# codyheiser/MILWRM

Hardware: AMD Instinct MI355X
Metric: pixels/sec (node) for preprocess+k-means fit+label, 30-ch MxIF k=8; %HBM peak (higher is better)
Workload: dtype f32 (fp64 accumulation)

## Files before the change

### include/milwrm_amd.h

```cpp
#ifndef MILWRM_AMD_H
#define MILWRM_AMD_H

#include <stddef.h>
#include <stdint.h>

#ifdef __cplusplus
extern "C" {
#endif

#define MW_OK 0
#define MW_EINVAL (-1)
#define MW_EHIP (-2)
#define MW_EUNSUPPORTED (-3)

#define MW_U8 0
#define MW_U16 1
#define MW_F32 2

int mw_version(void);
const char* mw_last_error(void);
int mw_stream_blocks(int64_t n);
int64_t mw_rows_per_block(int64_t n);

size_t mw_nz_stats_ws_bytes(int64_t n_pix, int C);
// ... 172 lines not shown
int mw_col_absmax(const float* d_X, int64_t S, int F, float* d_out, void* stream);
int mw_col_absmax_acc(const float* d_X, int64_t S, int F, float* d_out, void* stream);

int mw_kmeans_fit_history(int64_t* out, int cap);

size_t mw_kmeans_fit_ws_bytes(int64_t S, int F, int k);
int mw_kmeans_fit(const float* d_X, int64_t S, int F, const double* h_mu,
                  const double* h_inv, const double* h_feature_var, const float* h_xmax,
                  int k, const double* h_init, uint32_t seed, int max_iter, double tol,
                  uint8_t* d_labels, double* h_centers, double* h_inertia, int* h_n_iter,
                  int64_t* h_init_idx, void* d_ws, size_t ws_bytes, void* stream);
int mw_kmeans_fit_async(const float* d_X, int64_t S, int F, const double* h_mu,
                        const double* h_inv, const double* h_feature_var, const float* h_xmax,
                        int k, const double* h_init, uint32_t seed, int max_iter, double tol,
                        uint8_t* d_labels, double* h_centers, int* h_n_iter, int64_t* h_init_idx,
                        void* d_ws, size_t ws_bytes, double* h_final_rec, int* h_inertia_exp,
                        void* stream);
int mw_kmeans_fit_async_moments(const float* d_X, int64_t S, int F, const double* h_mu,
                                const double* h_inv, const double* h_feature_var, const float* h_xmax,
                                int k, const double* h_init, uint32_t seed, int max_iter, double tol,
                                uint8_t* d_labels, double* h_centers, int* h_n_iter, int64_t* h_init_idx,
                                void* d_ws, size_t ws_bytes, double* h_final_rec, int* h_inertia_exp,
                                int n_seg, const mw_kpp_seg* h_segs, void* stream);

int mw_lloyd_fits(const float* d_X, int64_t S, int F, const float* d_a32, const float* d_b32,
                  const int32_t* d_qexp, const float* h_a32, const float* h_b32,
                  const int32_t* h_qexp, const float* h_xmax, const double* h_mu,
                  const double* h_inv, int n, const int* h_k, const double* h_init,
                  uint8_t* const* d_labels, float* const* d_ub, float* const* d_lb,
                  void* const* d_ws, float* d_par, double* d_out, int max_iter, double tol,
                  int first_kind, int queue_kind, double queue_below, int dense_min,
                  int nobound, double* h_centers, double* h_inertia, int* h_n_iter,
                  int64_t* h_hist, int hist_cap, int* h_hist_len, double* h_timing,
                  void* stream);

typedef struct mw_fit_comm {
  void* ctx;
  int world;
  int rank;
  int64_t rows_total;
  int64_t row_offset;
  double* d_msg;
  int64_t msg_len;
  int (*all_reduce_sum)(void* ctx, int64_t off, int64_t n, void* stream);
  int (*all_gather)(void* ctx, int64_t in_off, int64_t n, int64_t out_off, void* stream);
} mw_fit_comm;
// ... 66 lines not shown
```

### milwrm_amd/_native.py

```python
from __future__ import annotations

import ctypes as C
import os
import threading

import torch

_HERE = os.path.dirname(os.path.abspath(__file__))
LIB_PATH = os.environ.get("MW_LIB") or os.path.join(_HERE, "libmilwrm_amd.so")

MW_U8, MW_U16, MW_F32 = 0, 1, 2
_EINVAL, _EHIP, _EUNSUP = -1, -2, -3

_lib = None
_lock = threading.Lock()

c_i64, c_i32, c_u32, c_u64 = C.c_int64, C.c_int, C.c_uint32, C.c_uint64
c_f32, c_sz, c_vp = C.c_float, C.c_size_t, C.c_void_p
c_dp = C.POINTER(C.c_double)

_PROTOS = {
    "mw_version": (c_i32, []),
    "mw_host_labels_f64": (c_i32, [c_vp, c_i64, c_vp, c_i32]),
    "mw_host_f32_to_f64": (c_i32, [c_vp, c_i64, c_vp, c_i32]),
# ... 52 lines not shown
                                 c_vp, c_vp, c_vp, c_vp, c_vp, c_vp, c_vp, c_vp, c_vp]),
    "mw_kpp_fold_rec_bytes": (c_sz, [c_i64, c_i32, c_i32]),
    "mw_kpp_fold_supported": (c_i32, [c_i32, c_i32, c_i32]),
    "mw_kmeans_fit_history": (c_i32, [c_vp, c_i32]),
    "mw_kpp_best_ptr": (c_vp, [c_vp, c_i64, c_i32]),
    "mw_kpp_pots": (c_i32, [c_vp, c_i64, c_i32, c_i32, c_vp, c_vp]),
    "mw_kpp_search": (c_i32, [c_vp, c_i64, c_i32, c_vp, c_i32, c_i32, c_i32, c_vp, c_vp, c_vp]),
    "mw_kpp_trial": (c_i32, [c_vp, c_i64, c_i32, c_vp, c_vp, c_i32, c_i32, c_vp, c_i32, c_vp, c_vp]),
    "mw_lloyd_ws_bytes": (c_sz, [c_i64, c_i32, c_i32]),
    "mw_lloyd_ws_bytes_kinds": (c_sz, [c_i64, c_i32, c_i32, c_i32]),
    "mw_lloyd_list_moved": (c_i32, [c_vp, c_vp, c_i64, c_i32, c_i32, c_vp, c_vp]),
    "mw_lloyd_rec_len": (c_i32, [c_i32, c_i32]),
    "mw_lloyd_pass": (c_i32, [c_vp, c_i64, c_i32, c_vp, c_vp, c_vp, c_i32, c_vp, c_i32, c_i32, c_vp]),
    "mw_col_absmax": (c_i32, [c_vp, c_i64, c_i32, c_vp, c_vp]),
    "mw_col_absmax_acc": (c_i32, [c_vp, c_i64, c_i32, c_vp, c_vp]),
    "mw_kmeans_fit_ws_bytes": (c_sz, [c_i64, c_i32, c_i32]),
    "mw_kmeans_fit": (c_i32, [c_vp, c_i64, c_i32, c_vp, c_vp, c_vp, c_vp, c_i32, c_vp, c_u32, c_i32,
                              C.c_double, c_vp, c_vp, c_vp, c_vp, c_vp, c_vp, c_sz, c_vp]),
    "mw_kmeans_fit_async": (c_i32, [c_vp, c_i64, c_i32, c_vp, c_vp, c_vp, c_vp, c_i32, c_vp, c_u32, c_i32,
                                    C.c_double, c_vp, c_vp, c_vp, c_vp, c_vp, c_sz, c_vp, c_vp, c_vp]),
    "mw_kmeans_fit_async_moments": (c_i32, [c_vp, c_i64, c_i32, c_vp, c_vp, c_vp, c_vp, c_i32, c_vp, c_u32, c_i32,
                                            C.c_double, c_vp, c_vp, c_vp, c_vp, c_vp, c_sz, c_vp, c_vp, c_i32,
                                            c_vp, c_vp]),
    "mw_lloyd_fits": (c_i32, [c_vp, c_i64, c_i32, c_vp, c_vp, c_vp, c_vp, c_vp, c_vp, c_vp, c_vp, c_vp,
                              c_i32, c_vp, c_vp, c_vp, c_vp, c_vp, c_vp, c_vp, c_vp, c_i32, C.c_double,
                              c_i32, c_i32, C.c_double, c_i32, c_i32, c_vp, c_vp, c_vp, c_vp, c_i32, c_vp,
                              c_vp, c_vp]),
    "mw_lloyd_fits_msg_len": (c_i64, [c_i64, c_i32, c_i32]),
    "mw_lloyd_fits_sharded": (c_i32, [c_vp, c_i64, c_i32, c_vp, c_vp, c_vp, c_vp, c_vp, c_vp, c_vp, c_vp, c_vp,
                                      c_i32, c_vp, c_vp, c_vp, c_vp, c_vp, c_vp, c_vp, c_vp, c_i32, C.c_double,
                                      c_i32, c_i32, C.c_double, c_i32, c_i32, c_vp, c_vp, c_vp, c_vp, c_i32,
                                      c_vp, c_vp, c_vp, c_vp]),
    "mw_farthest_ws_bytes": (c_sz, [c_i64]),
    "mw_farthest": (c_i32, [c_vp, c_i64, c_i32, c_vp, c_vp, c_vp, c_i32, c_vp, c_i32, c_vp, c_vp, c_vp, c_vp]),
    "mw_assign_ws_bytes": (c_sz, [c_i64, c_i32]),
    "mw_assign_conf": (c_i32, [c_vp, c_i32, c_vp, c_i32, c_vp, c_vp, c_vp, c_i32, c_vp, c_i64, c_vp, c_vp, c_vp, c_vp]),
    "mw_assign_reduce": (c_i32, [c_vp, c_i64, c_i32, c_vp, c_vp]),
    "mw_domain_sse_ws_bytes": (c_sz, [c_i64, c_i32, c_i32]),
    "mw_domain_sse_out_len": (c_i32, [c_i32, c_i32]),
    "mw_domain_sse": (c_i32, [c_vp, c_i32, c_vp, c_i32, c_vp, c_vp, c_vp, c_vp, c_vp, c_i32, c_i32, c_vp,
                              c_i64, c_vp, c_i32, c_vp, c_vp]),
    "mw_domain_sse_f64": (c_i32, [c_vp, c_i32, c_vp, c_i32, c_vp, c_vp, c_vp, c_vp, c_vp, c_i32, c_i32, c_vp,
                                  c_i64, c_vp, c_i32, c_vp, c_vp]),
    "mw_neighbor_mean": (c_i32, [c_vp, c_vp, c_i64, c_vp, c_i32, c_vp, c_vp]),
    "mw_col_stats_rows": (c_i32, [c_vp, c_i64, c_i32, c_vp, c_vp]),
    "mw_col_stats_absmax": (c_i32, [c_vp, c_i64, c_i32, c_vp, c_i32, c_vp]),
# ... 101 lines not shown
```

### milwrm_amd/csrc/fit.cpp

```cpp
#include <hip/hip_runtime.h>

#include <algorithm>
#include <chrono>
#include <cmath>
#include <cstring>
#include <limits>
#include <vector>

#include "common.h"

#pragma clang fp contract(off)

namespace mw {
void mt_init_genrand(uint32_t seed, uint32_t* mt);
void mt_regen(uint32_t* mt);

namespace {

struct LegacyRandom {
  uint32_t mt[624];
  int pos = 624;
  explicit LegacyRandom(uint32_t seed) { mt_init_genrand(seed, mt); }
  uint32_t next() {
    if (pos >= 624) { mt_regen(mt); pos = 0; }
    uint32_t y = mt[pos++];
    y ^= y >> 11;
    y ^= (y << 7) & 0x9D2C5680u;
    y ^= (y << 15) & 0xEFC60000u;
    y ^= y >> 18;
    return y;
  }
  double sample() {
    const uint32_t a = next() >> 5, b = next() >> 6;
    return (a * 67108864.0 + b) / 9007199254740992.0;
  }
};

double np_sum(const double* a, int64_t n) {
// ... 287 lines not shown
    return (e && e[0] == '0') ? 2 : 4;
  }();
  return q;
}
static FitLayout fit_layout(int64_t S, int F, int k) {
  const int T = 2 + (int)std::log((double)(k < 1 ? 1 : k));
  FitLayout L;
  L.small = 0;
  L.par = fal(64 * 4 * 4 + 64 * 8 * 2 + 64 * 64 * 8 + 64 * 8 * 2 + 130 * 8 + 64 * 8);
  L.ub = L.par + fal(((size_t)k * F + 2 * k) * 4);
  L.lb = L.ub + fal((size_t)S * 4);
  L.lws = L.lb + fal((size_t)S * 4);
  L.out = L.lws + fal(std::max(mw_lloyd_ws_bytes_kinds(S, k, F, lloyd_queue_kind() == 4),
                               mw_kpp_fold_rec_bytes(S, k, F)));
  L.big = L.out + fal((size_t)2 * mw_lloyd_rec_len(k, F) * 8);
  size_t big = mw_gather_ws_bytes(S, F);
  if (T <= 8) big = std::max(big, mw_kpp_ws_bytes(S, T));
  big = std::max(big, mw_farthest_ws_bytes(S));
  L.fold = L.big + fal(big);
  L.total = L.fold + fal(8192) + fal((size_t)S);
  return L;
}

}
}

using namespace mw;

extern "C" size_t mw_kmeans_fit_ws_bytes(int64_t S, int F, int k) {
  if (S <= 0 || F < 1 || F > 64 || k < 1 || k > 64) return 0;
  return fit_layout(S, F, k).total;
}

static int kmeans_fit_impl(const float* d_X, int64_t S, int F, const double* h_mu, const double* h_inv,
                           const double* h_feature_var, const float* h_xmax, int k, const double* h_init,
                           uint32_t seed, int max_iter, double tol, uint8_t* d_labels, double* h_centers,
                           double* h_inertia, int* h_n_iter, int64_t* h_init_idx, void* d_ws, size_t ws_bytes,
                           double* h_final_rec, int* h_inertia_exp, void* stream, int n_seg = 0,
                           const mw_kpp_seg* h_segs = nullptr);

static thread_local std::vector<int64_t> fit_hist;

extern "C" int mw_kmeans_fit_history(int64_t* out, int cap) {
  const int n = (int)(fit_hist.size() / 4);
  if (out)
    for (int i = 0; i < std::min(n, cap) * 4; ++i) out[i] = fit_hist[i];
  return n;
}

extern "C" int mw_kmeans_fit(const float* d_X, int64_t S, int F, const double* h_mu,
                             const double* h_inv, const double* h_feature_var, const float* h_xmax,
                             int k, const double* h_init, uint32_t seed, int max_iter, double tol,
                             uint8_t* d_labels, double* h_centers, double* h_inertia, int* h_n_iter,
                             int64_t* h_init_idx, void* d_ws, size_t ws_bytes, void* stream) {
  return kmeans_fit_impl(d_X, S, F, h_mu, h_inv, h_feature_var, h_xmax, k, h_init, seed, max_iter, tol,
                         d_labels, h_centers, h_inertia, h_n_iter, h_init_idx, d_ws, ws_bytes, nullptr, nullptr,
                         stream);
}

extern "C" int mw_kmeans_fit_async(const float* d_X, int64_t S, int F, const double* h_mu,
                                   const double* h_inv, const double* h_feature_var, const float* h_xmax,
                                   int k, const double* h_init, uint32_t seed, int max_iter, double tol,
// ... 2 lines not shown
                                   void* stream) {
  MW_CHECK_ARG(h_final_rec && h_inertia_exp, "mw_kmeans_fit_async: null final-record pointer");
  double unused = 0.0;
  return kmeans_fit_impl(d_X, S, F, h_mu, h_inv, h_feature_var, h_xmax, k, h_init, seed, max_iter, tol,
                         d_labels, h_centers, &unused, h_n_iter, h_init_idx, d_ws, ws_bytes, h_final_rec,
                         h_inertia_exp, stream);
}

extern "C" int mw_kmeans_fit_async_moments(const float* d_X, int64_t S, int F, const double* h_mu,
                                           const double* h_inv, const double* h_feature_var,
                                           const float* h_xmax, int k, const double* h_init, uint32_t seed,
                                           int max_iter, double tol, uint8_t* d_labels, double* h_centers,
                                           int* h_n_iter, int64_t* h_init_idx, void* d_ws, size_t ws_bytes,
                                           double* h_final_rec, int* h_inertia_exp, int n_seg,
                                           const mw_kpp_seg* h_segs, void* stream) {
  MW_CHECK_ARG(h_final_rec && h_inertia_exp, "mw_kmeans_fit_async_moments: null final-record pointer");
  MW_CHECK_ARG(n_seg == 0 || h_segs, "mw_kmeans_fit_async_moments: null segments");
  double unused = 0.0;
  return kmeans_fit_impl(d_X, S, F, h_mu, h_inv, h_feature_var, h_xmax, k, h_init, seed, max_iter, tol,
                         d_labels, h_centers, &unused, h_n_iter, h_init_idx, d_ws, ws_bytes, h_final_rec,
                         h_inertia_exp, stream, n_seg, h_segs);
}

static int kmeans_fit_impl(const float* d_X, int64_t S, int F, const double* h_mu, const double* h_inv,
                           const double* h_feature_var, const float* h_xmax, int k, const double* h_init,
                           uint32_t seed, int max_iter, double tol, uint8_t* d_labels, double* h_centers,
                           double* h_inertia, int* h_n_iter, int64_t* h_init_idx, void* d_ws, size_t ws_bytes,
                           double* h_final_rec, int* h_inertia_exp, void* stream, int n_seg,
                           const mw_kpp_seg* h_segs) {
  MW_CHECK_ARG(d_X && h_mu && h_inv && d_labels && h_centers && h_inertia && h_n_iter,
               "mw_kmeans_fit: null pointer");
  MW_CHECK_ARG(F >= 1 && F <= 64, "mw_kmeans_fit: F=%d outside [1, 64]", F);
  MW_CHECK_ARG(k >= 1 && k <= 64, "mw_kmeans_fit: n_clusters=%d outside [1, 64]", k);
  MW_CHECK_ARG(S >= k, "mw_kmeans_fit: n_samples=%lld should be >= n_clusters=%d", (long long)S, k);
  MW_CHECK_ARG(max_iter >= 1 && tol >= 0.0, "mw_kmeans_fit: bad max_iter / tol");
  const int T = 2 + (int)std::log((double)k);
  MW_CHECK_ARG(h_init || T <= 8, "mw_kmeans_fit: n_local_trials > 8");
  const FitLayout L = fit_layout(S, F, k);
  MW_CHECK_ARG(!d_ws || ws_bytes >= L.total, "mw_kmeans_fit: workspace %zu < %zu bytes", ws_bytes,
               L.total);
  hipStream_t st = as_stream(stream);
  DevBuf own;
  if (!d_ws) {
    MW_TRY(dev_alloc<char>(own, L.total));
    d_ws = own.p;
  }
  char* base = static_cast<char*>(d_ws);

  Fit fit;
  fit.S = S;
  fit.F = F;
  fit.k = k;
// ... 92 lines not shown

  std::vector<double> centers((size_t)k * F);
  if (h_init) {
    std::memcpy(centers.data(), h_init, centers.size() * sizeof(double));
  } else {
    LegacyRandom rs(seed);
    const double u0 = rs.sample();
    const int64_t first = first_center_index(S, u0);
    const bool moments = n_seg > 0 && k >= 2;
    std::vector<double> u(T);
    if (moments) {
      for (int t = 0; t < T; ++t) u[t] = rs.sample();
      MW_TRY(mw_kpp_init_moments(d_X, S, F, d_mu, d_inv, d_X + first * F, u.data(), T, n_seg, h_segs, big, st));
    } else {
      MW_TRY(mw_kpp_init(d_X, S, F, d_mu, d_inv, d_X + first * F, T, big, st));
    }
    for (int c = moments ? 2 : 1; c < k; ++c) {
      for (int t = 0; t < T; ++t) u[t] = rs.sample();
      if (fold && c == k - 1)
        MW_TRY(mw_kpp_step_fold(d_X, S, F, d_mu, d_inv, c, u.data(), T, big, first, fit.a32, fit.b32, fit.qexp,
                                d_labels, fit.ub, fit.lb, d_moved, base + L.fold, reinterpret_cast<double*>(fit.ws),
                                fit.out + fit.rl, st));
      else
        MW_TRY(mw_kpp_step(d_X, S, F, d_mu, d_inv, c, u.data(), T, big, st));
    }
    MW_TRY(mw_kpp_indices(big, S, T, k, d_idx, st));
    std::vector<int64_t> idx(k);
    if (fit.scaled_rows_dev(d_idx, first, k, h_mu, h_inv, reinterpret_cast<float*>(d_c64), centers,
                            idx.data()) == MW_OK) {
      if (h_init_idx) std::memcpy(h_init_idx, idx.data(), k * sizeof(int64_t));
    } else {
      MW_HIP(hipMemcpyAsync(idx.data(), d_idx, k * 8, hipMemcpyDeviceToHost, st));
      MW_HIP(hipStreamSynchronize(st));
      idx[0] = first;
      MW_TRY(fit.scaled_rows(idx.data(), k, h_mu, h_inv, centers));
      if (h_init_idx) std::memcpy(h_init_idx, idx.data(), k * sizeof(int64_t));
    }
  }

  fit_hist.clear();
  if (!fold) MW_HIP(hipMemsetAsync(d_labels, 255, (size_t)S, st));
  std::vector<int64_t> q_hi((size_t)k * F, 0), q_lo((size_t)k * F, 0), count(k, 0);
  std::vector<double> rec, cnew((size_t)k * F), weight(k), tmp(std::max(F, k));
  int64_t last_recomputed = -1;
  int n_iter = 0;
  bool done = false, strict = false;
  for (int it = 0; it < max_iter && !done; ++it) {
// ... 84 lines not shown
      } else {
        for (int f = 0; f < F; ++f) cnew[(size_t)j * F + f] = cnew[(size_t)amax * F + f];
      }
    }
    std::vector<double> shift2(k);
    for (int j = 0; j < k; ++j) {
      for (int f = 0; f < F; ++f) {
        const double d = cnew[(size_t)j * F + f] - centers[(size_t)j * F + f];
        tmp[f] = d * d;
      }
      const double sh = std::sqrt(np_sum(tmp.data(), F));
      shift2[j] = sh * sh;
    }
    centers.swap(cnew);
    n_iter = it + 1;
    if (changed == 0) {
      strict = done = true;
    } else if (np_sum(shift2.data(), k) <= tol_abs) {
      done = true;
    }
  }
  if (!done) n_iter = max_iter;

  std::vector<double> xs2(F), cn(k);
  for (int f = 0; f < F; ++f) {
    const double v = std::fabs(fit.a64[f]) * (double)xmax[f] + std::fabs(fit.b64[f]);
    xs2[f] = v * v;
  }
  const double xnorm = std::sqrt(np_sum(xs2.data(), F));
  double cmax = 0.0;
  for (int j = 0; j < k; ++j) {
    for (int f = 0; f < F; ++f) tmp[f] = centers[(size_t)j * F + f] * centers[(size_t)j * F + f];
    const double v = std::sqrt(np_sum(tmp.data(), F));
    cmax = j == 0 ? v : std::max(cmax, v);
  }
  const double xc = xnorm + cmax;
  const int iexp = exp_below(xc * xc * 1.01);
  MW_TRY(fit.upload(centers));
  fit_hist.insert(fit_hist.end(), {(int64_t)(strict ? 12 : 11), -1, -1, S});
  *h_n_iter = n_iter;
  std::memcpy(h_centers, centers.data(), centers.size() * sizeof(double));
  if (h_final_rec && !own.p && pinned_staging()) {
    MW_TRY(fit.pass_async(strict ? 2 : 1, 0, iexp, h_final_rec));
    *h_inertia_exp = iexp;
    hipEvent_t ev;
    MW_HIP(hipEventCreateWithFlags(&ev, hipEventDisableTiming));
    MW_HIP(hipEventRecord(ev, st));
    pin_busy = ev;
    *h_inertia = std::numeric_limits<double>::quiet_NaN();
    return MW_OK;
  }
  MW_TRY(fit.pass(strict ? 2 : 1, 0, iexp, rec));
  const double* tail = rec.data() + fit.rl - 4;
  *h_inertia = (tail[2] * 4294967296.0 + tail[3]) * std::ldexp(1.0, -iexp);
  if (h_final_rec) {
    std::memcpy(h_final_rec, rec.data(), (size_t)fit.rl * sizeof(double));
    *h_inertia_exp = iexp;
  }
  return MW_OK;
}

namespace mw {
namespace {

constexpr int kFitsMaxPerLaunch = 24;
constexpr int kKindFirst = 0, kKindTile = 1, kKindDense = 5;

struct FitsFit {
  int k = 0;
  std::vector<double> centers;
  std::vector<float> prev32;
  bool have_prev = false;
  std::vector<int64_t> q_hi, q_lo, count;
  bool done = false, strict = false, bounds_ok = true;
  int n_iter = 0;
  double drift_max = 0.0, prev_dmax = 0.0;
  int iexp = 0;
  std::vector<int64_t> hist;
};

void fits_tables(FitsFit& fs, int F, bool nobound, float* h) {
  const int k = fs.k;
// ... 557 lines not shown
```

### milwrm_amd/csrc/kpp.hip

```cpp
#include <math.h>
#include <stdlib.h>

#include "kmeans_common.h"

namespace mw {

constexpr int kKppTab = 64 + 64 * 8 + 64 + 8;
constexpr int kKppTabBytes = kKppTab * 8;

static inline size_t al256(size_t x) { return (x + 255) & ~(size_t)255; }

constexpr int kMomSegs = 16;
constexpr int kMomBlocks = 16384;
struct KppLayout {
  size_t cur, bsum, tsum, tab, st, mom, total;
  int G;
  int64_t NTL;
};
static KppLayout kpp_layout(int64_t S, int T) {
  KppLayout L;
  L.G = kblocks(S);
  L.NTL = (S + 63) / 64;
  L.cur = 0;
  L.bsum = al256((size_t)S * sizeof(double));
// ... 129 lines not shown
      t0 = n0;
      t1 = n1;
    }
  } else {
#pragma unroll 4
    for (int f = 0; f < fend; ++f) feat((double)xr[f], f);
  }
#pragma unroll
  for (int c = 0; c < T; ++c) {
    const double e = fma(-2.0, dot[c], xx) + tb[640 + c];
    d[c] = e > 0.0 ? e : 0.0;
  }
  if (MODE >= 2) {
    const double e = fma(-2.0, dotp, xx) + tcc;
    dp = e > 0.0 ? e : 0.0;
  }
}

template <int FMAX, int T, int MODE>
__global__ void __launch_bounds__(256, FMAX == 64 ? 2 : 4) kpp_pass_kernel(
    const float* __restrict__ X, int64_t S, int F, const double* __restrict__ tab,
    const double* __restrict__ tab_prev, const int* __restrict__ best, int best_val,
    double* __restrict__ cur, int64_t R, int64_t NTL, double* __restrict__ bsum_new,
    double* __restrict__ tsum_new) {
  constexpr int NV = FMAX / 4;
  extern __shared__ __attribute__((aligned(16))) char smem[];
  double* s_red = reinterpret_cast<double*>(smem);
  const int t = threadIdx.x, lane = t & 63, nw = blockDim.x >> 6;
  const int wid = __builtin_amdgcn_readfirstlane(t >> 6);
  constexpr bool FS = FMAX == 64;
  const int tstride = FS ? 64 * F + 4 : 64 * FMAX;
  const int fend = FS ? F : FMAX;
  float* s_tile = reinterpret_cast<float*>(smem + 64) + (size_t)wid * tstride;
  if (FS && lane < 4) s_tile[64 * F + lane] = 0.f;

  const int64_t lo = (int64_t)blockIdx.x * R, hi = min(S, lo + R);
  const int ntile = hi > lo ? (int)((hi - lo + 63) / 64) : 0;
  const int64_t total = S * (int64_t)F, n4 = total >> 2;
  const __amdgpu_buffer_rsrc_t rx = make_rsrc(X + lo * F, (S - lo) * F * 4);
  constexpr bool LOADS_CUR = MODE == 1 || MODE == 2;
  const __amdgpu_buffer_rsrc_t rc = make_rsrc(cur + lo, LOADS_CUR ? (hi - lo) * 8 : 0);
  const int tile_bytes = 64 * F * 4;
  double acc[T];
#pragma unroll
  for (int c = 0; c < T; ++c) acc[c] = 0.0;
  __syncthreads();

// ... 78 lines not shown
          t0 = n0;
          t1 = n1;
        }
      }
    } else {
#pragma unroll 4
      for (int f = 0; f < fend; ++f) feat((double)xr[f], f);
    }
#pragma unroll
    for (int c = 0; c < T; ++c) {
      const double e = fma(-2.0, dot[c], xx) + tb[640 + c];
      d[c] = e > 0.0 ? e : 0.0;
    }
    if (MODE >= 2) {
      const double e = fma(-2.0, dotp, xx) + tcc;
      dp = e > 0.0 ? e : 0.0;
    }
    }
    const bool valid = lane < nrow;
    const int64_t row = r0 + lane;
    if (MODE == 0) cd = d[0];
    if (MODE == 2) cd = cd < dp ? cd : dp;
    if (MODE == 3) cd = dp;
    if (MODE != 1 && valid) cur[row] = cd;
    double mv[T];
#pragma unroll
    for (int c = 0; c < T; ++c) {
      const double m = MODE == 0 ? d[0] : (cd < d[c] ? cd : d[c]);
      mv[c] = valid ? m : 0.0;
      acc[c] += mv[c];
    }
    kpp_tile_sums<T>(mv, lane, tsum_new + (r0 >> 6), NTL);
  }
#pragma unroll
  for (int c = 0; c < T; ++c) {
    const double tot = block_sum(acc[c], s_red);
    if (t == 0) bsum_new[(size_t)c * gridDim.x + blockIdx.x] = tot;
  }
}

struct KppFoldArg {
  const float* a32;
  const float* b32;
  const int* qexp;
  const f2v* gT;
  int kb;
  uint8_t* labels;
// ... 488 lines not shown
  }
  for (int o = 32; o > 0; o >>= 1) blk = min(blk, __shfl_xor(blk, o, 64));
  const double base = blk > 0 ? s[blk - 1] : 0.0;
  const int64_t lo = (int64_t)blk * R, hi = min(S, lo + R);
  int64_t idx = kpp_find_row(lo, hi, tsum_cur + (size_t)b * NTL + (lo >> 6), base, rv, lane, s_row[w],
                                   [&](int64_t row) {
                                     double a = cur[row];
                                     if (has_pend) {
                                       const double dp = kpp_dist_row(X + row * F, F, tab_prev, b);
                                       a = a < dp ? a : dp;
                                     }
                                     return a;
                                   });
  if (lane == 0) {
    if (idx > S - 1) idx = S - 1;
    if (idx < 0) idx = 0;
    cand[w] = idx;
  }
}

static int kpp_pass_launch(const float* X, int64_t S, int F, const double* mu, const double* inv,
                           const KppPtrs& p, int c, const int* best, int best_val,
                           const int64_t* cand, const float* rows, int T, int64_t* chosen_reset,
                           hipStream_t s, bool c0_pending = false) {
  double* tab = p.tab_of(c);
  hipLaunchKernelGGL(kpp_prep_kernel, dim3(1), dim3(512), 0, s, X, F, mu, inv, cand, rows, T, tab,
                     chosen_reset);
  MW_LAUNCH_CHECK();
  const int FM = F <= 8 ? 8 : F <= 16 ? 16 : F <= 32 ? 32 : 64;
  const size_t lds = 64 + (size_t)4 * (FM == 64 ? 64 * F + 4 : 64 * FM) * sizeof(float);
  const int mode = c == 0 ? 0 : c == 1 ? (c0_pending ? 3 : 1) : 2;
  const double* tab_prev = c >= 1 ? p.tab_of(c - 1) : nullptr;
  double* bs = p.bsum_of(c, T);
  double* tsm = p.tsum_of(c, T);
  const int64_t R = krows(S);
#define MW_KP(FMV, TV, MV)                                                                      \
  hipLaunchKernelGGL((kpp_pass_kernel<FMV, TV, MV>), dim3(p.L.G), dim3(256), lds, s, X, S, F, tab, \
                     tab_prev, best, best_val, p.cur, R, p.L.NTL, bs, tsm)
#define MW_KPM(FMV, TV) \
  if (mode == 1) MW_KP(FMV, TV, 1); else if (mode == 3) MW_KP(FMV, TV, 3); else MW_KP(FMV, TV, 2);
#define MW_KPT(FMV)                                                                        \
  if (mode == 0) { MW_KP(FMV, 1, 0); }                                                     \
  else switch (T) {                                                                        \
    case 1: MW_KPM(FMV, 1) break; case 2: MW_KPM(FMV, 2) break;                            \
    case 3: MW_KPM(FMV, 3) break; case 4: MW_KPM(FMV, 4) break;                            \
    case 5: MW_KPM(FMV, 5) break; case 6: MW_KPM(FMV, 6) break;                            \
    case 7: MW_KPM(FMV, 7) break; default: MW_KPM(FMV, 8) break;                           \
  }
  if (FM == 8) { MW_KPT(8) }
  else if (FM == 16) { MW_KPT(16) }
  else if (FM == 32) { MW_KPT(32) }
  else { MW_KPT(64) }
#undef MW_KPT
#undef MW_KPM
#undef MW_KP
  MW_LAUNCH_CHECK();
  return MW_OK;
}

static int kpp_search_launch(const float* X, int64_t S, int F, const KppPtrs& p, int c, int n_cur,
                             const double* u, int T, int n_tgt, int best_given,
                             const double* rv_given, hipStream_t s) {
  hipLaunchKernelGGL(kpp_search_kernel, dim3(1), dim3(1024), 0, s, X, F, p.cur, p.tab_of(c - 1),
                     c >= 2 ? 1 : 0, p.bsum_of(c - 1, T), p.tsum_of(c - 1, T), n_cur, S, p.L.G,
                     krows(S), p.L.NTL, best_given >= 0 ? 0 : c - 1, u[0], u[1], u[2], u[3], u[4],
                     u[5], u[6], u[7], n_tgt, p.cand, p.chosen, p.best, best_given, rv_given);
  MW_LAUNCH_CHECK();
  return MW_OK;
}

}

using namespace mw;

extern "C" {

size_t mw_kpp_ws_bytes(int64_t S, int T) { return kpp_layout(S, T).total; }

int mw_kpp_init(const float* d_X, int64_t S, int F, const double* d_mu, const double* d_inv,
                const float* d_center_row, int T, void* d_ws, void* stream) {
  MW_CHECK_ARG(d_X && d_mu && d_inv && d_ws && d_center_row, "mw_kpp_init: null pointer");
  MW_CHECK_ARG(S > 0 && F > 0 && F <= 64, "mw_kpp_init: bad shape (F <= 64)");
  MW_CHECK_ARG(T >= 1 && T <= 8, "mw_kpp_init: n_local_trials must be in [1, 8]");
  const KppPtrs p = kpp_ptrs(d_ws, S, T);
  return kpp_pass_launch(d_X, S, F, d_mu, d_inv, p, 0, nullptr, 0, nullptr, d_center_row, 1,
                         p.chosen, as_stream(stream));
}

void mw_kpp_ws_sections(int64_t S, int T, int64_t* out) {
  const KppLayout L = kpp_layout(S, T);
  out[0] = (int64_t)L.cur;
// ... 40 lines not shown
  for (int i = 0; i < T; ++i) us.u[i] = h_u[i];
  double* tab0 = p.tab_of(0);
  hipLaunchKernelGGL(kpp_prep_kernel, dim3(1), dim3(512), 0, s, d_X, F, d_mu, d_inv,
                     (const int64_t*)nullptr, d_center_row, 1, tab0, p.chosen);
  hipLaunchKernelGGL(kpp_mom_sums_kernel, dim3(1), dim3(1024), 0, s, m, F, d_inv, d_center_row, p.msum,
                     p.mscan);
  MW_LAUNCH_CHECK();
  const int64_t tiles = (rmax + 63) / 64;
  const int nsub = (int)std::min<int64_t>(64, std::max<int64_t>(1, (tiles + 3) / 4));
  double* ts0 = p.tsum_of(0, T);
  hipLaunchKernelGGL(kpp_mom_tiles_kernel, dim3(nsub, T), dim3(256), 0, s, d_X, F, tab0, m, p.mscan, us,
                     p.L.NTL, ts0);
  hipLaunchKernelGGL(kpp_mom_search_kernel, dim3(1), dim3(64 * T), 0, s, d_X, F, tab0, m, p.mscan, us, S,
                     p.L.NTL, ts0, p.cand, p.best);
  MW_LAUNCH_CHECK();
  return kpp_pass_launch(d_X, S, F, d_mu, d_inv, p, 1, nullptr, 0, p.cand, nullptr, T, nullptr, s, true);
}

int mw_kpp_step(const float* d_X, int64_t S, int F, const double* d_mu, const double* d_inv, int c,
                const double* h_u, int T, void* d_ws, void* stream) {
  MW_CHECK_ARG(d_X && d_mu && d_inv && d_ws && h_u, "mw_kpp_step: null pointer");
  MW_CHECK_ARG(c >= 1 && c < 256, "mw_kpp_step: center index %d out of range", c);
  MW_CHECK_ARG(T >= 1 && T <= 8 && F > 0 && F <= 64, "mw_kpp_step: T in [1,8], F <= 64 required");
  const KppPtrs p = kpp_ptrs(d_ws, S, T);
  double u[8] = {0, 0, 0, 0, 0, 0, 0, 0};
  for (int i = 0; i < T; ++i) u[i] = h_u[i];
  hipStream_t s = as_stream(stream);
  const int rc = kpp_search_launch(d_X, S, F, p, c, c == 1 ? 1 : T, u, T, T, -1, nullptr, s);
  if (rc != MW_OK) return rc;
  return kpp_pass_launch(d_X, S, F, d_mu, d_inv, p, c, p.best, 0, p.cand, nullptr, T, nullptr, s);
}

int mw_kpp_fold_supported(int k, int F, int T) {
  return k >= 3 && k <= 16 && T >= 1 && T <= 4 && F >= 1 && F <= 32 && kpp_fold_lds(k, F) <= kFoldLdsMax;
}

size_t mw_kpp_fold_rec_bytes(int64_t S, int k, int F) {
  return (size_t)kblocks(S) * lloyd_rec(k, F) * sizeof(double);
}

const int* mw_kpp_best_ptr(const void* d_ws, int64_t S, int T) { return kpp_ptrs(d_ws, S, T).best; }

int mw_kpp_step_fold(const float* d_X, int64_t S, int F, const double* d_mu, const double* d_inv, int c,
                     const double* h_u, int T, void* d_ws, int64_t first, const float* d_a32,
                     const float* d_b32, const int32_t* d_qexp, uint8_t* d_labels, float* d_ub, float* d_lb,
                     uint8_t* d_moved, void* d_centers_img, double* d_rec, double* d_rec_out, void* stream) {
  MW_CHECK_ARG(d_X && d_mu && d_inv && d_ws && h_u && d_a32 && d_b32 && d_qexp && d_labels && d_ub && d_lb &&
                   d_moved && d_centers_img && d_rec && d_rec_out,
               "mw_kpp_step_fold: null pointer");
  MW_CHECK_ARG(c >= 2 && mw_kpp_fold_supported(c + 1, F, T) && first >= 0 && first < S,
               "mw_kpp_step_fold: unsupported (k=%d F=%d T=%d: mw_kpp_fold_supported)", c + 1, F, T);
  const KppPtrs p = kpp_ptrs(d_ws, S, T);
  double u[8] = {0, 0, 0, 0, 0, 0, 0, 0};
// ... 92 lines not shown
```

### milwrm_amd/kmeans.py

```python
from __future__ import annotations

import ctypes as C
import os
import warnings

import numpy as np
import torch

from . import _native as N
from . import device as D
from . import profiling
from .rng import as_random_state, first_center_index, kpp_draws


class DeviceRows:

    def __init__(self, X: torch.Tensor, mu=None, inv=None, feature_var=None, xmax_local=None):
        assert X.dtype == torch.float32 and X.dim() == 2 and X.is_contiguous()
        self.X = X
        self.S, self.F = X.shape
        self.mu = np.zeros(self.F) if mu is None else np.asarray(mu, dtype=np.float64)
        self.inv = np.ones(self.F) if inv is None else np.asarray(inv, dtype=np.float64)
        self.a_host = self.inv.astype(np.float32)
        self.b_host = (-self.mu * self.inv).astype(np.float32)
# ... 117 lines not shown
        if self.with_mean:
            X -= self.mean_
        if self.with_std:
            X /= self.scale_
        return X

    def fit_transform(self, X, y=None):
        return self.fit(X).transform(X)

    def inverse_transform(self, X, copy=None):
        X = np.array(X, dtype=np.float64, copy=True)
        if self.with_std:
            X *= self.scale_
        if self.with_mean:
            X += self.mean_
        return X

    def affine(self):
        return self.mean_.copy(), 1.0 / self.scale_



KPP_INIT_USED = {"moments": 0, "pass": 0}


def _kmeans_plusplus_device(rows: DeviceRows, k: int, random_state, n_local_trials=None, moments=False):
    S, F = rows.S, rows.F
    T = 2 + int(np.log(k)) if n_local_trials is None else int(n_local_trials)
    u0, steps = kpp_draws(random_state, k, T)
    first = first_center_index(S, u0)
    ws = D.WS.get("kpp", N.query("mw_kpp_ws_bytes", S, T))
    st = D.stream()
    segs = rows.moment_segments() if moments and k >= 2 else None
    if segs is not None:
        u = np.ascontiguousarray(steps[0], dtype=np.float64)
        with profiling.timed("kpp_step", S * (F * 4 + 8 * T)):
            N.call("mw_kpp_init_moments", D.P(rows.X), S, F, D.P(rows.mu64), D.P(rows.inv64),
                   D.P(rows.X) + int(first) * F * 4, u.ctypes.data, T, segs[0], C.addressof(segs[1]),
                   D.P(ws), st)
        KPP_INIT_USED["moments"] += 1
    else:
        with profiling.timed("kpp_init", S * (F * 4 + 8)):
            N.call("mw_kpp_init", D.P(rows.X), S, F, D.P(rows.mu64), D.P(rows.inv64),
                   D.P(rows.X) + int(first) * F * 4, T, D.P(ws), st)
        KPP_INIT_USED["pass"] += 1
    for c in range(1 if segs is None else 2, k):
# ... 509 lines not shown
            lrows.qexp = rows.qexp
    res = lloyd_fits(lrows, inits, max_iters.pop(), tols.pop(), False, comm)
    del lrows
    for km, (labels, inertia, centers, n_iter) in zip(models, res):
        if perm is not None:
            back = torch.empty_like(labels)
            back[perm] = labels
            labels = back
        km._set_fitted(rows, labels, inertia, centers, n_iter)
    return models


class _Inertia:

    def __init__(self, event, rec: torch.Tensor, iexp: int):
        self.event, self.rec, self.iexp = event, rec, int(iexp)

    def value(self) -> float:
        self.event.synchronize()
        r = self.rec.numpy()
        return float((r[-2] * 4294967296.0 + r[-1]) * 2.0 ** -self.iexp)


class KMeans:

    def __init__(self, n_clusters=8, *, init="k-means++", n_init="auto", max_iter=300, tol=1e-4,
                 verbose=0, random_state=None, copy_x=True, algorithm="lloyd"):
        self.n_clusters = n_clusters
        self.init = init
        self.n_init = n_init
        self.max_iter = max_iter
        self.tol = tol
        self.verbose = verbose
        self.random_state = random_state
        self.copy_x = copy_x
        self.algorithm = algorithm

    def get_params(self, deep=True):
        return dict(n_clusters=self.n_clusters, init=self.init, n_init=self.n_init,
                    max_iter=self.max_iter, tol=self.tol, verbose=self.verbose,
                    random_state=self.random_state, copy_x=self.copy_x, algorithm=self.algorithm)

    def set_params(self, **p):
        for k, v in p.items():
            setattr(self, k, v)
        return self
# ... 49 lines not shown
                                     f"match the number of clusters {k} / features {rows.F}.")
                self.init_indices_ = None
            elif init == "k-means++":
                seeded = n_init == 1 and isinstance(self.random_state, (int, np.integer)) \
                    and not isinstance(self.random_state, bool)
                centers0, self.init_indices_ = self._kpp(rows, self.random_state if seeded else rs(),
                                                         comm, moments=True)
            elif init == "random":
                if comm.sharded():
                    raise NotImplementedError("init='random' with sharded rows")
                seeds = rs().choice(rows.S, size=k, replace=False,
                                  p=np.full(rows.S, 1.0 / rows.S))
                centers0, self.init_indices_ = rows.scaled_rows(seeds), seeds
            elif callable(init):
                raise NotImplementedError("callable init")
            else:
                raise ValueError(f"init should be 'k-means++', 'random' or an array, got {init!r}")
            labels, inertia, centers, n_iter = lloyd_device(rows, centers0, self.max_iter,
                                                            self._tol, bool(self.verbose), comm)
            if best is None or inertia < best[1]:
                best = (labels, inertia, centers, n_iter)
        return self._set_fitted(rows, *best)

    def _fit_c(self, rows, k, init):
        S, F = rows.S, rows.F
        mu = np.ascontiguousarray(rows.mu, dtype=np.float64)
        inv = np.ascontiguousarray(rows.inv, dtype=np.float64)
        var = np.ascontiguousarray(rows.feature_var(), dtype=np.float64) if self.tol else None
        xmax = None if rows._xmax_local is None else np.ascontiguousarray(rows._xmax_local, np.float32)
        c0 = None
        if init is not None:
            c0 = np.ascontiguousarray(np.array(init, dtype=np.float64))
            if c0.shape != (k, F):
                raise ValueError(f"The shape of the initial centers {c0.shape} does not "
                                 f"match the number of clusters {k} / features {F}.")
        labels = torch.empty(S, dtype=torch.uint8, device=rows.X.device)
        centers = np.zeros((k, F))
        n_iter, iexp = C.c_int(), C.c_int()
        idx = np.full(k, -1, dtype=np.int64)
        nb = N.query("mw_kmeans_fit_ws_bytes", S, F, k)
        from .stream import RESIDENCY

        RESIDENCY.release(nb + S + (64 << 20))
        ws = D.WS.get("kfit", nb)
        rec = torch.empty(N.query("mw_lloyd_rec_len", k, F), dtype=torch.float64, pin_memory=True)
        segs = rows.moment_segments() if c0 is None and k >= 2 else None
        with profiling.timed("kmeans_fit", 0):
            N.call("mw_kmeans_fit_async_moments", D.P(rows.X), S, F, mu.ctypes.data, inv.ctypes.data,
                   None if var is None else var.ctypes.data,
                   None if xmax is None else xmax.ctypes.data, k,
                   None if c0 is None else c0.ctypes.data,
                   0 if c0 is not None else int(self.random_state),
                   int(self.max_iter), float(self.tol or 0.0), D.P(labels), centers.ctypes.data,
                   C.addressof(n_iter), idx.ctypes.data, D.P(ws), ws.numel(), rec.data_ptr(),
                   C.addressof(iexp), 0 if segs is None else segs[0],
                   None if segs is None else C.addressof(segs[1]), D.stream())
            done = torch.cuda.Event()
            done.record()
        if c0 is None:
            KPP_INIT_USED["moments" if segs is not None else "pass"] += 1
        self.init_indices_ = None if c0 is not None else idx
        return labels, _Inertia(done, rec, iexp.value), centers, n_iter.value

    def _kpp(self, rows, rs, comm, moments=False):
        if comm.sharded():
            KPP_INIT_USED["pass"] += 1
            return comm.kpp(rows, int(self.n_clusters), rs)
        return _kmeans_plusplus_device(rows, int(self.n_clusters), rs, moments=moments)

    def _set_fitted(self, rows, labels, inertia, centers, n_iter):
        self._labels_dev = labels
        self.cluster_centers_ = centers
        self._inertia = inertia
        self.n_iter_ = n_iter
        self.n_features_in_ = rows.F
        self._n_features_out = int(self.n_clusters)
        self._labels_host = None
        return self

    @property
    def inertia_(self) -> float:
        if isinstance(self._inertia, _Inertia):
            self._inertia = self._inertia.value()
        return self._inertia

    @inertia_.setter
    def inertia_(self, v):
        self._inertia = v

    @property
    def labels_(self):
        if self._labels_host is None:
            self._labels_host = self._labels_dev.cpu().numpy().astype(np.int32)
        return self._labels_host

    def fit_predict(self, X, y=None, sample_weight=None):
        return self.fit(X, sample_weight=sample_weight).labels_

    def predict(self, X):
        from .assign import assign_rows

        X = np.asarray(X, dtype=np.float64)
        if X.ndim != 2 or X.shape[1] != self.cluster_centers_.shape[1]:
            raise ValueError("X has the wrong shape")
# ... 3 lines not shown
```

Measured before the change: 6.429 billion.

## Defer final labeling pass until labels or inertia are accessed

Splits k-means fit into a deferred fit that returns centers without running the final assignment/inertia pass, and a separate finish call that runs it lazily when labels or inertia are first read. It also skips storing the per-row distance array on the last k-means++ step, since nothing reads it afterwards. This removes a full pass over the data when callers never read labels or inertia, and saves one write stream during init. The cost is extra host-side bookkeeping. If the column absmax is missing it now has to be computed on the device and copied back to the host before the fit, which adds a synchronisation.

```diff
diff --git a/include/milwrm_amd.h b/include/milwrm_amd.h
--- a/include/milwrm_amd.h
+++ b/include/milwrm_amd.h
@@ -218,6 +218,17 @@
                                 uint8_t* d_labels, double* h_centers, int* h_n_iter, int64_t* h_init_idx,
                                 void* d_ws, size_t ws_bytes, double* h_final_rec, int* h_inertia_exp,
                                 int n_seg, const mw_kpp_seg* h_segs, void* stream);
+int mw_kmeans_fit_deferred(const float* d_X, int64_t S, int F, const double* h_mu,
+                           const double* h_inv, const double* h_feature_var, const float* h_xmax,
+                           int k, const double* h_init, uint32_t seed, int max_iter, double tol,
+                           uint8_t* d_labels, double* h_centers, int* h_n_iter, int64_t* h_init_idx,
+                           void* d_ws, size_t ws_bytes, int n_seg, const mw_kpp_seg* h_segs,
+                           int* h_strict, void* stream);
+size_t mw_kmeans_fit_finish_ws_bytes(int64_t S, int F, int k);
+int mw_kmeans_fit_finish(const float* d_X, int64_t S, int F, const double* h_mu, const double* h_inv,
+                         const float* h_xmax, int k, const double* h_centers, int strict,
+                         uint8_t* d_labels, void* d_ws, size_t ws_bytes, double* h_final_rec,
+                         int* h_inertia_exp, void* stream);
 
 int mw_lloyd_fits(const float* d_X, int64_t S, int F, const float* d_a32, const float* d_b32,
                   const int32_t* d_qexp, const float* h_a32, const float* h_b32,
diff --git a/milwrm_amd/_native.py b/milwrm_amd/_native.py
--- a/milwrm_amd/_native.py
+++ b/milwrm_amd/_native.py
@@ -98,6 +98,11 @@
     "mw_kmeans_fit_async_moments": (c_i32, [c_vp, c_i64, c_i32, c_vp, c_vp, c_vp, c_vp, c_i32, c_vp, c_u32, c_i32,
                                             C.c_double, c_vp, c_vp, c_vp, c_vp, c_vp, c_sz, c_vp, c_vp, c_i32,
                                             c_vp, c_vp]),
+    "mw_kmeans_fit_deferred": (c_i32, [c_vp, c_i64, c_i32, c_vp, c_vp, c_vp, c_vp, c_i32, c_vp, c_u32, c_i32,
+                                       C.c_double, c_vp, c_vp, c_vp, c_vp, c_vp, c_sz, c_i32, c_vp, c_vp, c_vp]),
+    "mw_kmeans_fit_finish_ws_bytes": (c_sz, [c_i64, c_i32, c_i32]),
+    "mw_kmeans_fit_finish": (c_i32, [c_vp, c_i64, c_i32, c_vp, c_vp, c_vp, c_i32, c_vp, c_i32, c_vp, c_vp, c_sz,
+                                     c_vp, c_vp, c_vp]),
     "mw_lloyd_fits": (c_i32, [c_vp, c_i64, c_i32, c_vp, c_vp, c_vp, c_vp, c_vp, c_vp, c_vp, c_vp, c_vp,
                               c_i32, c_vp, c_vp, c_vp, c_vp, c_vp, c_vp, c_vp, c_vp, c_i32, C.c_double,
                               c_i32, c_i32, C.c_double, c_i32, c_i32, c_vp, c_vp, c_vp, c_vp, c_i32, c_vp,
diff --git a/milwrm_amd/csrc/fit.cpp b/milwrm_amd/csrc/fit.cpp
--- a/milwrm_amd/csrc/fit.cpp
+++ b/milwrm_amd/csrc/fit.cpp
@@ -14,6 +14,8 @@
 namespace mw {
 void mt_init_genrand(uint32_t seed, uint32_t* mt);
 void mt_regen(uint32_t* mt);
+int kpp_step(const float* d_X, int64_t S, int F, const double* d_mu, const double* d_inv, int c,
+             const double* h_u, int T, void* d_ws, void* stream, bool store_cur);
 
 namespace {
 
@@ -347,6 +349,58 @@
   return L;
 }
 
+struct FinishLayout {
+  size_t small, par, lws, out, total;
+};
+static FinishLayout finish_layout(int64_t S, int F, int k) {
+  FinishLayout L;
+  L.small = 0;
+  L.par = fal(64 * 4 * 3);
+  L.lws = L.par + fal(((size_t)k * F + 2 * k) * 4);
+  L.out = L.lws + fal(mw_lloyd_ws_bytes_kinds(S, k, F, 0));
+  L.total = L.out + fal((size_t)mw_lloyd_rec_len(k, F) * 8);
+  return L;
+}
+
+static int fit_tail(Fit& fit, const float* xmax, const std::vector<double>& centers, bool strict,
+                    bool async_end, double* h_inertia, double* h_final_rec, int* h_inertia_exp) {
+  const int F = fit.F, k = fit.k;
+  std::vector<double> xs2(F), tmp(std::max(F, k));
+  for (int f = 0; f < F; ++f) {
+    const double v = std::fabs(fit.a64[f]) * (double)xmax[f] + std::fabs(fit.b64[f]);
+    xs2[f] = v * v;
+  }
+  const double xnorm = std::sqrt(np_sum(xs2.data(), F));
+  double cmax = 0.0;
+  for (int j = 0; j < k; ++j) {
+    for (int f = 0; f < F; ++f) tmp[f] = centers[(size_t)j * F + f] * centers[(size_t)j * F + f];
+    const double v = std::sqrt(np_sum(tmp.data(), F));
+    cmax = j == 0 ? v : std::max(cmax, v);
+  }
+  const double xc = xnorm + cmax;
+  const int iexp = exp_below(xc * xc * 1.01);
+  MW_TRY(fit.upload(centers));
+  if (async_end && h_final_rec && pinned_staging()) {
+    MW_TRY(fit.pass_async(strict ? 2 : 1, 0, iexp, h_final_rec));
+    *h_inertia_exp = iexp;
+    hipEvent_t ev;
+    MW_HIP(hipEventCreateWithFlags(&ev, hipEventDisableTiming));
+    MW_HIP(hipEventRecord(ev, fit.st));
+    pin_busy = ev;
+    *h_inertia = std::numeric_limits<double>::quiet_NaN();
+    return MW_OK;
+  }
+  std::vector<double> rec;
+  MW_TRY(fit.pass(strict ? 2 : 1, 0, iexp, rec));
+  const double* tail = rec.data() + fit.rl - 4;
+  *h_inertia = (tail[2] * 4294967296.0 + tail[3]) * std::ldexp(1.0, -iexp);
+  if (h_final_rec) {
+    std::memcpy(h_final_rec, rec.data(), (size_t)fit.rl * sizeof(double));
+    *h_inertia_exp = iexp;
+  }
+  return MW_OK;
+}
+
 }
 }
 
@@ -362,7 +416,7 @@
                            uint32_t seed, int max_iter, double tol, uint8_t* d_labels, double* h_centers,
                            double* h_inertia, int* h_n_iter, int64_t* h_init_idx, void* d_ws, size_t ws_bytes,
                            double* h_final_rec, int* h_inertia_exp, void* stream, int n_seg = 0,
-                           const mw_kpp_seg* h_segs = nullptr);
+                           const mw_kpp_seg* h_segs = nullptr, int* h_strict = nullptr);
 
 static thread_local std::vector<int64_t> fit_hist;
 
@@ -411,12 +465,83 @@
                          h_inertia_exp, stream, n_seg, h_segs);
 }
 
+extern "C" int mw_kmeans_fit_deferred(const float* d_X, int64_t S, int F, const double* h_mu,
+                                      const double* h_inv, const double* h_feature_var, const float* h_xmax,
+                                      int k, const double* h_init, uint32_t seed, int max_iter, double tol,
+                                      uint8_t* d_labels, double* h_centers, int* h_n_iter,
+                                      int64_t* h_init_idx, void* d_ws, size_t ws_bytes, int n_seg,
+                                      const mw_kpp_seg* h_segs, int* h_strict, void* stream) {
+  MW_CHECK_ARG(h_strict, "mw_kmeans_fit_deferred: null h_strict");
+  MW_CHECK_ARG(n_seg == 0 || h_segs, "mw_kmeans_fit_deferred: null segments");
+  double unused = 0.0;
+  return kmeans_fit_impl(d_X, S, F, h_mu, h_inv, h_feature_var, h_xmax, k, h_init, seed, max_iter, tol,
+                         d_labels, h_centers, &unused, h_n_iter, h_init_idx, d_ws, ws_bytes, nullptr, nullptr,
+                         stream, n_seg, h_segs, h_strict);
+}
+
+extern "C" size_t mw_kmeans_fit_finish_ws_bytes(int64_t S, int F, int k) {
+  if (S <= 0 || F < 1 || F > 64 || k < 1 || k > 64) return 0;
+  return finish_layout(S, F, k).total;
+}
+
+extern "C" int mw_kmeans_fit_finish(const float* d_X, int64_t S, int F, const double* h_mu,
+                                    const double* h_inv, const float* h_xmax, int k, const double* h_centers,
+                                    int strict, uint8_t* d_labels, void* d_ws, size_t ws_bytes,
+                                    double* h_final_rec, int* h_inertia_exp, void* stream) {
+  MW_CHECK_ARG(d_X && h_mu && h_inv && h_xmax && h_centers && d_labels && d_ws && h_final_rec && h_inertia_exp,
+               "mw_kmeans_fit_finish: null pointer");
+  MW_CHECK_ARG(F >= 1 && F <= 64, "mw_kmeans_fit_finish: F=%d outside [1, 64]", F);
+  MW_CHECK_ARG(k >= 1 && k <= 64, "mw_kmeans_fit_finish: n_clusters=%d outside [1, 64]", k);
+  MW_CHECK_ARG(S >= k, "mw_kmeans_fit_finish: n_samples=%lld should be >= n_clusters=%d", (long long)S, k);
+  const FinishLayout L = finish_layout(S, F, k);
+  MW_CHECK_ARG(ws_bytes >= L.total, "mw_kmeans_fit_finish: workspace %zu < %zu bytes", ws_bytes, L.total);
+  char* base = static_cast<char*>(d_ws);
+  Fit fit;
+  fit.S = S;
+  fit.F = F;
+  fit.k = k;
+  fit.st = as_stream(stream);
+  fit.X = d_X;
+  fit.rl = mw_lloyd_rec_len(k, F);
+  fit.a32 = reinterpret_cast<float*>(base + L.small);
+  fit.b32 = fit.a32 + 64;
+  fit.qexp = reinterpret_cast<int32_t*>(fit.b32 + 64);
+  fit.par = reinterpret_cast<float*>(base + L.par);
+  fit.ub = fit.lb = nullptr;
+  fit.ws = base + L.lws;
+  fit.out = reinterpret_cast<double*>(base + L.out);
+  fit.labels = d_labels;
+  fit.a64.resize(F);
+  fit.b64.resize(F);
+  std::vector<char> blk(64 * 4 * 3, 0);
+  float* fa = reinterpret_cast<float*>(blk.data());
+  int32_t* qi = reinterpret_cast<int32_t*>(fa + 128);
+  for (int f = 0; f < F; ++f) {
+    fa[f] = (float)h_inv[f];
+    fa[64 + f] = (float)(-h_mu[f] * h_inv[f]);
+    qi[f] = exp_below((double)h_xmax[f]);
+    fit.a64[f] = (double)fa[f];
+    fit.b64[f] = (double)fa[64 + f];
+  }
+  char* pin = pinned_staging();
+  const void* src = blk.data();
+  if (pin) {
+    std::memcpy(pin + kPinSetup, blk.data(), blk.size());
+    src = pin + kPinSetup;
+  }
+  MW_HIP(hipMemcpyAsync(fit.a32, src, blk.size(), hipMemcpyHostToDevice, fit.st));
+  if (!pin) MW_HIP(hipStreamSynchronize(fit.st));
+  const std::vector<double> centers(h_centers, h_centers + (size_t)k * F);
+  double unused = 0.0;
+  return fit_tail(fit, h_xmax, centers, strict != 0, true, &unused, h_final_rec, h_inertia_exp);
+}
+
 static int kmeans_fit_impl(const float* d_X, int64_t S, int F, const double* h_mu, const double* h_inv,
                            const double* h_feature_var, const float* h_xmax, int k, const double* h_init,
                            uint32_t seed, int max_iter, double tol, uint8_t* d_labels, double* h_centers,
                            double* h_inertia, int* h_n_iter, int64_t* h_init_idx, void* d_ws, size_t ws_bytes,
                            double* h_final_rec, int* h_inertia_exp, void* stream, int n_seg,
-                           const mw_kpp_seg* h_segs) {
+                           const mw_kpp_seg* h_segs, int* h_strict) {
   MW_CHECK_ARG(d_X && h_mu && h_inv && d_labels && h_centers && h_inertia && h_n_iter,
                "mw_kmeans_fit: null pointer");
   MW_CHECK_ARG(F >= 1 && F <= 64, "mw_kmeans_fit: F=%d outside [1, 64]", F);
@@ -555,7 +680,7 @@
                                 d_labels, fit.ub, fit.lb, d_moved, base + L.fold, reinterpret_cast<double*>(fit.ws),
                                 fit.out + fit.rl, st));
       else
-        MW_TRY(mw_kpp_step(d_X, S, F, d_mu, d_inv, c, u.data(), T, big, st));
+        MW_TRY(kpp_step(d_X, S, F, d_mu, d_inv, c, u.data(), T, big, st, c < k - 1));
     }
     MW_TRY(mw_kpp_indices(big, S, T, k, d_idx, st));
     std::vector<int64_t> idx(k);
@@ -686,42 +811,14 @@
   }
   if (!done) n_iter = max_iter;
 
-  std::vector<double> xs2(F), cn(k);
-  for (int f = 0; f < F; ++f) {
-    const double v = std::fabs(fit.a64[f]) * (double)xmax[f] + std::fabs(fit.b64[f]);
-    xs2[f] = v * v;
-  }
-  const double xnorm = std::sqrt(np_sum(xs2.data(), F));
-  double cmax = 0.0;
-  for (int j = 0; j < k; ++j) {
-    for (int f = 0; f < F; ++f) tmp[f] = centers[(size_t)j * F + f] * centers[(size_t)j * F + f];
-    const double v = std::sqrt(np_sum(tmp.data(), F));
-    cmax = j == 0 ? v : std::max(cmax, v);
-  }
-  const double xc = xnorm + cmax;
-  const int iexp = exp_below(xc * xc * 1.01);
-  MW_TRY(fit.upload(centers));
-  fit_hist.insert(fit_hist.end(), {(int64_t)(strict ? 12 : 11), -1, -1, S});
   *h_n_iter = n_iter;
   std::memcpy(h_centers, centers.data(), centers.size() * sizeof(double));
-  if (h_final_rec && !own.p && pinned_staging()) {
-    MW_TRY(fit.pass_async(strict ? 2 : 1, 0, iexp, h_final_rec));
-    *h_inertia_exp = iexp;
-    hipEvent_t ev;
-    MW_HIP(hipEventCreateWithFlags(&ev, hipEventDisableTiming));
-    MW_HIP(hipEventRecord(ev, st));
-    pin_busy = ev;
-    *h_inertia = std::numeric_limits<double>::quiet_NaN();
+  if (h_strict) {
+    *h_strict = strict ? 1 : 0;
     return MW_OK;
   }
-  MW_TRY(fit.pass(strict ? 2 : 1, 0, iexp, rec));
-  const double* tail = rec.data() + fit.rl - 4;
-  *h_inertia = (tail[2] * 4294967296.0 + tail[3]) * std::ldexp(1.0, -iexp);
-  if (h_final_rec) {
-    std::memcpy(h_final_rec, rec.data(), (size_t)fit.rl * sizeof(double));
-    *h_inertia_exp = iexp;
-  }
-  return MW_OK;
+  fit_hist.insert(fit_hist.end(), {(int64_t)(strict ? 12 : 11), -1, -1, S});
+  return fit_tail(fit, xmax.data(), centers, strict, !own.p, h_inertia, h_final_rec, h_inertia_exp);
 }
 
 namespace mw {
diff --git a/milwrm_amd/csrc/kpp.hip b/milwrm_amd/csrc/kpp.hip
--- a/milwrm_amd/csrc/kpp.hip
+++ b/milwrm_amd/csrc/kpp.hip
@@ -175,7 +175,7 @@
     const float* __restrict__ X, int64_t S, int F, const double* __restrict__ tab,
     const double* __restrict__ tab_prev, const int* __restrict__ best, int best_val,
     double* __restrict__ cur, int64_t R, int64_t NTL, double* __restrict__ bsum_new,
-    double* __restrict__ tsum_new) {
+    double* __restrict__ tsum_new, int store_cur) {
   constexpr int NV = FMAX / 4;
   extern __shared__ __attribute__((aligned(16))) char smem[];
   double* s_red = reinterpret_cast<double*>(smem);
@@ -300,7 +300,7 @@
     if (MODE == 0) cd = d[0];
     if (MODE == 2) cd = cd < dp ? cd : dp;
     if (MODE == 3) cd = dp;
-    if (MODE != 1 && valid) cur[row] = cd;
+    if (MODE != 1 && valid && store_cur) cur[row] = cd;
     double mv[T];
 #pragma unroll
     for (int c = 0; c < T; ++c) {
@@ -835,7 +835,7 @@
 static int kpp_pass_launch(const float* X, int64_t S, int F, const double* mu, const double* inv,
                            const KppPtrs& p, int c, const int* best, int best_val,
                            const int64_t* cand, const float* rows, int T, int64_t* chosen_reset,
-                           hipStream_t s, bool c0_pending = false) {
+                           hipStream_t s, bool c0_pending = false, bool store_cur = true) {
   double* tab = p.tab_of(c);
   hipLaunchKernelGGL(kpp_prep_kernel, dim3(1), dim3(512), 0, s, X, F, mu, inv, cand, rows, T, tab,
                      chosen_reset);
@@ -849,7 +849,7 @@
   const int64_t R = krows(S);
 #define MW_KP(FMV, TV, MV)                                                                      \
   hipLaunchKernelGGL((kpp_pass_kernel<FMV, TV, MV>), dim3(p.L.G), dim3(256), lds, s, X, S, F, tab, \
-                     tab_prev, best, best_val, p.cur, R, p.L.NTL, bs, tsm)
+                     tab_prev, best, best_val, p.cur, R, p.L.NTL, bs, tsm, store_cur ? 1 : 0)
 #define MW_KPM(FMV, TV) \
   if (mode == 1) MW_KP(FMV, TV, 1); else if (mode == 3) MW_KP(FMV, TV, 3); else MW_KP(FMV, TV, 2);
 #define MW_KPT(FMV)                                                                        \
@@ -880,6 +880,18 @@
                      u[5], u[6], u[7], n_tgt, p.cand, p.chosen, p.best, best_given, rv_given);
   MW_LAUNCH_CHECK();
   return MW_OK;
+}
+
+int kpp_step(const float* d_X, int64_t S, int F, const double* d_mu, const double* d_inv, int c,
+             const double* h_u, int T, void* d_ws, void* stream, bool store_cur) {
+  const KppPtrs p = kpp_ptrs(d_ws, S, T);
+  double u[8] = {0, 0, 0, 0, 0, 0, 0, 0};
+  for (int i = 0; i < T; ++i) u[i] = h_u[i];
+  hipStream_t s = as_stream(stream);
+  const int rc = kpp_search_launch(d_X, S, F, p, c, c == 1 ? 1 : T, u, T, T, -1, nullptr, s);
+  if (rc != MW_OK) return rc;
+  return kpp_pass_launch(d_X, S, F, d_mu, d_inv, p, c, p.best, 0, p.cand, nullptr, T, nullptr, s, false,
+                         store_cur);
 }
 
 }
@@ -966,13 +978,7 @@
   MW_CHECK_ARG(d_X && d_mu && d_inv && d_ws && h_u, "mw_kpp_step: null pointer");
   MW_CHECK_ARG(c >= 1 && c < 256, "mw_kpp_step: center index %d out of range", c);
   MW_CHECK_ARG(T >= 1 && T <= 8 && F > 0 && F <= 64, "mw_kpp_step: T in [1,8], F <= 64 required");
-  const KppPtrs p = kpp_ptrs(d_ws, S, T);
-  double u[8] = {0, 0, 0, 0, 0, 0, 0, 0};
-  for (int i = 0; i < T; ++i) u[i] = h_u[i];
-  hipStream_t s = as_stream(stream);
-  const int rc = kpp_search_launch(d_X, S, F, p, c, c == 1 ? 1 : T, u, T, T, -1, nullptr, s);
-  if (rc != MW_OK) return rc;
-  return kpp_pass_launch(d_X, S, F, d_mu, d_inv, p, c, p.best, 0, p.cand, nullptr, T, nullptr, s);
+  return kpp_step(d_X, S, F, d_mu, d_inv, c, h_u, T, d_ws, stream, true);
 }
 
 int mw_kpp_fold_supported(int k, int F, int T) {
diff --git a/milwrm_amd/kmeans.py b/milwrm_amd/kmeans.py
--- a/milwrm_amd/kmeans.py
+++ b/milwrm_amd/kmeans.py
@@ -163,6 +163,7 @@
 
 
 KPP_INIT_USED = {"moments": 0, "pass": 0}
+FIT_FINISH_USED = {"finish": 0}
 
 
 def _kmeans_plusplus_device(rows: DeviceRows, k: int, random_state, n_local_trials=None, moments=False):
@@ -718,6 +719,13 @@
         return float((r[-2] * 4294967296.0 + r[-1]) * 2.0 ** -self.iexp)
 
 
+class _Deferred:
+
+    def __init__(self, X: torch.Tensor, mu, inv, xmax, strict: bool, centers):
+        self.X, self.mu, self.inv, self.xmax, self.strict = X, mu, inv, xmax, bool(strict)
+        self.centers = np.array(centers, dtype=np.float64)
+
+
 class KMeans:
 
     def __init__(self, n_clusters=8, *, init="k-means++", n_init="auto", max_iter=300, tol=1e-4,
@@ -813,7 +821,7 @@
                 best = (labels, inertia, centers, n_iter)
         return self._set_fitted(rows, *best)
 
-    def _fit_c(self, rows, k, init):
+    def _fit_c(self, rows, k, init, defer=True):
         S, F = rows.S, rows.F
         mu = np.ascontiguousarray(rows.mu, dtype=np.float64)
         inv = np.ascontiguousarray(rows.inv, dtype=np.float64)
@@ -834,8 +842,27 @@
 
         RESIDENCY.release(nb + S + (64 << 20))
         ws = D.WS.get("kfit", nb)
+        segs = rows.moment_segments() if c0 is None and k >= 2 else None
+        if defer:
+            if xmax is None:
+                m = torch.empty(F, dtype=torch.float32, device=rows.X.device)
+                N.call("mw_col_absmax", D.P(rows.X), S, F, D.P(m), D.stream())
+                xmax = np.ascontiguousarray(D.d2h(m), np.float32)
+            strict = C.c_int()
+            with profiling.timed("kmeans_fit", 0):
+                N.call("mw_kmeans_fit_deferred", D.P(rows.X), S, F, mu.ctypes.data, inv.ctypes.data,
+                       None if var is None else var.ctypes.data, xmax.ctypes.data, k,
+                       None if c0 is None else c0.ctypes.data,
+                       0 if c0 is not None else int(self.random_state),
+                       int(self.max_iter), float(self.tol or 0.0), D.P(labels), centers.ctypes.data,
+                       C.addressof(n_iter), idx.ctypes.data, D.P(ws), ws.numel(),
+                       0 if segs is None else segs[0], None if segs is None else C.addressof(segs[1]),
+                       C.addressof(strict), D.stream())
+            if c0 is None:
+                KPP_INIT_USED["moments" if segs is not None else "pass"] += 1
+            self.init_indices_ = None if c0 is not None else idx
+            return labels, _Deferred(rows.X, mu, inv, xmax, strict.value != 0, centers), centers, n_iter.value
         rec = torch.empty(N.query("mw_lloyd_rec_len", k, F), dtype=torch.float64, pin_memory=True)
-        segs = rows.moment_segments() if c0 is None and k >= 2 else None
         with profiling.timed("kmeans_fit", 0):
             N.call("mw_kmeans_fit_async_moments", D.P(rows.X), S, F, mu.ctypes.data, inv.ctypes.data,
                    None if var is None else var.ctypes.data,
@@ -860,17 +887,53 @@
         return _kmeans_plusplus_device(rows, int(self.n_clusters), rs, moments=moments)
 
     def _set_fitted(self, rows, labels, inertia, centers, n_iter):
-        self._labels_dev = labels
+        self._labels_buf = labels
         self.cluster_centers_ = centers
-        self._inertia = inertia
+        self._pending = inertia if isinstance(inertia, _Deferred) else None
+        self._inertia = None if self._pending is not None else inertia
         self.n_iter_ = n_iter
         self.n_features_in_ = rows.F
         self._n_features_out = int(self.n_clusters)
         self._labels_host = None
         return self
 
+    def _finish(self):
+        d = getattr(self, "_pending", None)
+        if d is None:
+            return
+        S, F = d.X.shape
+        centers = d.centers
+        k = centers.shape[0]
+        ws = D.WS.get("kfit_finish", N.query("mw_kmeans_fit_finish_ws_bytes", S, F, k))
+        rec = torch.empty(N.query("mw_lloyd_rec_len", k, F), dtype=torch.float64, pin_memory=True)
+        iexp = C.c_int()
+        with profiling.timed("kmeans_finish", S * F * 4):
+            N.call("mw_kmeans_fit_finish", D.P(d.X), S, F, d.mu.ctypes.data, d.inv.ctypes.data,
+                   d.xmax.ctypes.data, k, centers.ctypes.data, int(d.strict), D.P(self._labels_buf), D.P(ws),
+                   ws.numel(), rec.data_ptr(), C.addressof(iexp), D.stream())
+            done = torch.cuda.Event()
+            done.record()
+        self._pending = None
+        FIT_FINISH_USED["finish"] += 1
+        if self._inertia is None:
+            self._inertia = _Inertia(done, rec, iexp.value)
+
+    def finalize(self):
+        self._finish()
+        return self
+
+    @property
+    def _labels_dev(self) -> torch.Tensor:
+        self._finish()
+        return self._labels_buf
+
+    @_labels_dev.setter
+    def _labels_dev(self, v):
+        self._labels_buf = v
+
     @property
     def inertia_(self) -> float:
+        self._finish()
         if isinstance(self._inertia, _Inertia):
             self._inertia = self._inertia.value()
         return self._inertia
```

After: 6.568 billion, median of 6. 2.2% higher.
